# DhayaaAnbajagane/Baryonification

Hardware: AMD Instinct MI355X
Metric: halos/sec for BaryonifyShell NSIDE=1024 (1000000-halo synthetic catalog) (higher is better)
Workload: dtype f64 throughout in the parity-grade mode: f64 ring-row geometry, f64 pair math with 1e-11 elementary functions (fp32 seeds + one Newton step), f64 LDS accumulation, pix_offsets stored as two f32 arrays (hi + lo), f64 regrid geometry, f64 map

## Files before the change

baryonification_amd/csrc/bfgx_api.hip:

```cpp
#include <hip/hip_runtime.h>
#include <cmath>
#include <cstdarg>
#include <cstdio>
#include <algorithm>
#include <climits>
#include <cstdint>
#include <cstdlib>
#include <chrono>
#include <cstring>
#include <functional>
#include <map>
#include <mutex>
#include <string>
#include <tuple>
#include <type_traits>
#include <vector>

#include "../../include/bfgx.h"

#include "bfgx_devmem.hpp"
#include "bfgx_tile_arena.hpp"
#include "bfgx_cosmo.hpp"
#include "bfgx_kernels.hpp"
#include "bfgx_scatter2.hpp"
// ... 65 lines not shown
    for (int d = 0; d < t.ndim; ++d) {
        if (t.n[d] < 2) return fail(BFGX_ERR_INVALID, "table axis %d needs >= 2 points", d);
        if (!t.axis[d]) return fail(BFGX_ERR_INVALID, "table axis %d pointer is NULL", d);
        for (int i = 1; i < t.n[d]; ++i)
            if (!(t.axis[d][i] > t.axis[d][i - 1]))
                return fail(BFGX_ERR_INVALID, "table axis %d must be strictly ascending", d);
    }
    double tot = 1.0;
    for (int d = 0; d < t.ndim; ++d) tot *= t.n[d];
    if (tot > 2.0e9) return fail(BFGX_ERR_INVALID, "table too large for 32-bit row offsets");
    return BFGX_OK;
}

}

struct bfgx_plan {
    int device = 0, num_cus = 256;
    hipStream_t stream = nullptr;
    int64_t nside = 0, max_halos = 0;
    Hpx hpx;
    DevModel model;
    DevList mem;
    HaloRec *recs = nullptr;
    RowSetX *rowsx = nullptr;
    int NC = 4;
    int algo = 1;
    bool blocking_growth = false;
    float *k0_work_est = nullptr;
    int32_t *k1_form = nullptr;
    int64_t k1_nhalos = 0;
    int k1_fluid = 1;
    Tiling tiling;
    TileArena arena;
    int32_t *tile_start = nullptr, *entries = nullptr, *overflow = nullptr;
    int32_t *entries_a = nullptr, *slow_list = nullptr, *slow_cnt = nullptr;
    int32_t entries_a_cap = 0;
    int32_t cnt_pad = 1;
    TileRef *tref = nullptr;
    FarList far;
    int32_t *regrid_lean = nullptr;
    int auto_acc = 0;
    double table_disp_pixels = 0.0;
    int32_t *tile_apron = nullptr;
    int band_reach = 1;
    int route_margin = 0;
    int64_t cat_blk_rows = 0, cat_blk_stride = 0;
    ScanScratch scan;
    bool fast_ok = false;
    RowRec *rowrec = nullptr;
    void *pairrec = nullptr;
    FbRec *fbrec = nullptr;
    const float *tab8f = nullptr;
    const double *tab8d = nullptr;
    unsigned long long *pair_total = nullptr;
    double *tile_sums = nullptr;
    std::vector<int32_t> band_tile0_host;
    int64_t capacity = 0;
    bool timing = false;
    std::vector<std::pair<hipEvent_t, hipEvent_t>> ev[BFGX_NUM_KERNELS];
    std::vector<std::pair<hipEvent_t, hipEvent_t>> ev_free;
};

namespace {

template <class Plan>
struct KernelTimerT {
// ... 122 lines not shown
    float *lo(const void *offsets, int64_t n) const { return split() ? (float *)offsets + 3 * (size_t)n : nullptr; }
    int acc() const { return kind == F32 ? BFGX_ACC_F32 : kind == F64 ? BFGX_ACC_F64 : BFGX_ACC_PARITY; }
};

static int disp_mode(const bfgx_plan *p, int acc, bool one_array, DispMode &m)
{
    if (!p) return fail(BFGX_ERR_INVALID, "NULL plan");
    if (acc != BFGX_ACC_AUTO && acc != BFGX_ACC_F32 && acc != BFGX_ACC_F64 && acc != BFGX_ACC_PARITY)
        return fail(BFGX_ERR_INVALID, "acc_f64 = %d: must be BFGX_ACC_AUTO (-1), 0 (f32), 1 (f64) or BFGX_ACC_PARITY (3)", acc);
    if (acc == BFGX_ACC_AUTO) acc = p->auto_acc;
    const bool parity = acc == BFGX_ACC_PARITY && use_fast(p);
    m.kind = acc == BFGX_ACC_F32 ? DispMode::F32 : (parity && !one_array) ? DispMode::SPLIT : DispMode::F64;
    return BFGX_OK;
}

struct PaintMode {
    enum Kind { F32, F64, MIXED } kind = F64;
    bool map_f64() const { return kind != F32; }
    bool k0_f64() const { return kind == F64; }
    bool pair_f32() const { return kind == MIXED; }
};

static int paint_mode(const bfgx_plan *p, int acc, PaintMode &m)
{
    if (!p) return fail(BFGX_ERR_INVALID, "NULL plan");
    if (acc < 0 || acc > 2) return fail(BFGX_ERR_INVALID, "acc_f64 must be 0, 1 or 2");
    m.kind = acc == 0 ? PaintMode::F32 : (acc == 2 && use_fast(p)) ? PaintMode::MIXED : PaintMode::F64;
    return BFGX_OK;
}

struct TileLaunch {
    float *offsets_lo = nullptr;
    bool paint_pair_f32 = false;
    float *omax = nullptr;
    int tile_lo = 0, tile_n = -1;
    int spread_tiles = -1;
};

static int launch_prep(bfgx_plan *p, const bfgx_catalog *c, int fallback4, bool bin, bool f64, bool rec_all)
{
    if (c->n == 0) return BFGX_OK;
    const unsigned grid = (unsigned)((c->n + 255) / 256);
    KernelTimer kt(p, BFGX_K_PREP);
    PrepOut o;
    std::memset(&o, 0, sizeof(o));
    o.rec = p->recs; o.rowsx = p->rowsx;
    o.fast = (bin && use_fast(p)) ? 1 : 0;
    o.rec_all = (rec_all || !o.fast) ? 1 : 0;
    o.rowrec = p->rowrec; o.pairrec = p->pairrec; o.fbrec = p->fbrec;
    if (bin) {
        o.tref = p->tref; o.cnt_a = p->arena.cnt_a_pad; o.cnt_b = p->arena.cnt_b;
        o.cnt_pad = p->cnt_pad;
        o.work_est = o.fast ? p->k0_work_est : nullptr;
        o.entries_a = p->entries_a; o.cap_a = p->entries_a_cap; o.slow_list = p->slow_list; o.slow_cnt = p->slow_cnt;
    }
    o.ncell_m = p->model.tab.n[1] - 1; o.nrm1 = p->model.tab.n[2] - 1;
    o.blk_rows = p->cat_blk_rows; o.blk_stride = p->cat_blk_stride;
    ExtraCols ex;
    for (int k = 0; k < BFGX_MAX_EXTRA; ++k) ex.p[k] = c->extra[k];
#define BFGX_PREP(NCV, REAL)                                                                                        \
    hipLaunchKernelGGL((halo_prep_kernel<NCV, REAL>), dim3(grid), dim3(256), 0, p->stream, p->model, p->hpx, c->n, c->M, c->z, \
                       c->ra, c->dec, ex, c->ln1pz, c->lnM, fallback4, p->tiling, o)
    if (p->NC == 4) { if (f64) BFGX_PREP(4, double); else BFGX_PREP(4, float); }
    else if (p->NC == 8) BFGX_PREP(8, float);
    else if (p->NC == 16) BFGX_PREP(16, float);
    else if (p->NC == 32) BFGX_PREP(32, float);
    else BFGX_PREP(64, float);
#undef BFGX_PREP
    HIP_TRY(hipGetLastError());
    return BFGX_OK;
}

static int launch_place(bfgx_plan *p, const bfgx_catalog *c)
{
    const unsigned grid = (unsigned)((c->n + 255) / 256);
    hipLaunchKernelGGL(tile_place_kernel, dim3(grid), dim3(256), 0, p->stream, p->hpx, p->tiling, c->n,
                       (const TileRef *)p->tref, (const int32_t *)p->tile_start, p->arena.cur_b, p->entries, p->capacity, p->overflow,
                       (const int32_t *)p->slow_list, (const int32_t *)p->slow_cnt);
    HIP_TRY(hipGetLastError());
    return BFGX_OK;
}

static int launch_prep_and_bin(bfgx_plan *p, const bfgx_catalog *c, int fallback4, bool f64)
{
    p->k1_nhalos = c->n;
    HIP_TRY(hipMemsetAsync(p->arena.base, 0, p->arena.zeroed_bytes, p->stream));
    if (int rc = launch_prep(p, c, fallback4, true, f64, false)) return rc;
    KernelTimer kt(p, BFGX_K_BIN);
    const int nt_i = p->tiling.ntiles, nsb = (nt_i + kScanTilesPerWg - 1) / kScanTilesPerWg;
    const int32_t *cnt = p->arena.cnt_b;
    if (nsb <= 1 || nsb > 1024) {
        hipLaunchKernelGGL(tile_scan_kernel, dim3(1), dim3(1024), 0, p->stream, nt_i, cnt, p->tile_start);
    } else {
        int32_t *tot = p->scan.block_tot, *off = p->scan.block_off;
        hipLaunchKernelGGL(tile_scan_part_kernel<0>, dim3(nsb), dim3(1024), 0, p->stream, nt_i, cnt, p->tile_start, tot, (const int32_t *)off);
        hipLaunchKernelGGL(tile_scan_blocks_kernel, dim3(1), dim3(1024), 0, p->stream, nsb, nt_i, (const int32_t *)tot, off, p->tile_start);
        hipLaunchKernelGGL(tile_scan_part_kernel<1>, dim3(nsb), dim3(1024), 0, p->stream, nt_i, cnt, p->tile_start, tot, (const int32_t *)off);
    }
    HIP_TRY(hipGetLastError());
    if (c->n > 0) if (int rc = launch_place(p, c)) return rc;
    return BFGX_OK;
}

template <int MODE, typename ACC>
static int launch_scatter(bfgx_plan *p, int64_t n, ACC *out, int64_t *counts)
{
    if (n == 0) return BFGX_OK;
    const unsigned grid = (unsigned)((n + kWavesPerBlock - 1) / kWavesPerBlock);
    KernelTimer kt(p, MODE == MODE_OFFSETS ? BFGX_K_OFFSETS : (MODE == MODE_PAINT ? BFGX_K_PAINT : BFGX_K_COUNT));
    hipLaunchKernelGGL((halo_scatter_kernel<MODE, ACC>), dim3(grid), dim3(kWave * kWavesPerBlock), 0, p->stream,
                       make_pair_table(p->model.tab), p->hpx, n, (const HaloRec *)p->recs, out, counts);
    HIP_TRY(hipGetLastError());
    return BFGX_OK;
}

template <int MODE, typename ACC, int NC>
static int launch_tile_scatter_nc(bfgx_plan *p, ACC *out, const TileLaunch &k)
{
    constexpr int NCOMP = (MODE == MODE_OFFSETS) ? 3 : 1;
    const size_t lds = tile_lds_bytes<NC>(p->tiling.BR, p->tiling.W, NCOMP);
    auto kern = tile_scatter_kernel<MODE, ACC, NC>;
    HIP_TRY(hipFuncSetAttribute((const void *)kern, hipFuncAttributeMaxDynamicSharedMemorySize, (int)lds));
    KernelTimer kt(p, MODE == MODE_OFFSETS ? BFGX_K_OFFSETS : (MODE == MODE_PAINT ? BFGX_K_PAINT : BFGX_K_COUNT));
    const int grid = k.tile_n < 0 ? p->tiling.ntiles : std::max(k.tile_n, 1);
    hipLaunchKernelGGL(kern, dim3(grid), dim3(kWave * kWavesPerBlock), lds, p->stream,
                       make_pair_table(p->model.tab), p->hpx, p->tiling, (const HaloRec *)p->recs, (const RowSetX *)p->rowsx,
                       (const int32_t *)p->tile_start, (const int32_t *)p->entries, p->capacity, out, p->pair_total,
                       (unsigned int *)k.omax, k.tile_lo, k.tile_n);
    HIP_TRY(hipGetLastError());
    return BFGX_OK;
}

template <int MODE, typename ACC, typename real, int PM = 0>
static int launch_tile_scatter2(bfgx_plan *p, ACC *out, const TileLaunch &k, ACC *out_lo = nullptr)
{
    constexpr int NCOMP = (MODE == MODE_OFFSETS) ? 3 : 1;
    constexpr int kNP = 1;
    const size_t lds = tile2_lds_bytes<real>(p->tiling.BR, p->tiling.W, NCOMP);
    auto kern = tile_scatter2_kernel<MODE, ACC, real, kNP, PM>;
    HIP_TRY(hipFuncSetAttribute((const void *)kern, hipFuncAttributeMaxDynamicSharedMemorySize, (int)lds));
    Tab8T<real> tb;
    tb.v = (sizeof(real) == 4) ? (const real *)p->tab8f : (const real *)p->tab8d;
    tb.r0 = (real)p->model.tab.r0; tb.r1 = (real)p->model.tab.r1; tb.inv_dr = (real)p->model.tab.inv_dr;
    tb.nr = p->model.tab.n[2]; tb._pad = 0;
    unsigned int *tile_counter = p->arena.tile_counter;
    const int ntodo = k.tile_n < 0 ? p->tiling.ntiles : std::max(k.tile_n, 1);
    KernelTimer kt(p, MODE == MODE_OFFSETS ? BFGX_K_OFFSETS : (MODE == MODE_PAINT ? BFGX_K_PAINT : BFGX_K_COUNT));
    int32_t *form = nullptr;
    if constexpr (MODE != MODE_COUNT) {
        const size_t ldsf = tile2f_lds_bytes<real>(p->tiling.BR, p->tiling.W, NCOMP);
        const bool eligible = p->k1_fluid && ldsf <= (size_t)160 * 1024 && p->tiling.BR <= kWave && ntodo >= 2 * p->num_cus;
        const int nspread = k.spread_tiles > 0 ? k.spread_tiles : ntodo;
        const bool dense = (double)p->k1_nhalos * (double)p->tiling.ntiles >= 6.0e5 * (double)nspread;
        const bool forced = p->k1_fluid == 2 && ldsf <= (size_t)160 * 1024 && p->tiling.BR <= kWave;
        if (eligible && !dense && !forced && p->k0_work_est && p->k1_nhalos > 0) {
            const int nblk = (int)((p->k1_nhalos + 255) / 256);
            hipLaunchKernelGGL(k1_form_kernel, dim3(1), dim3(1024), 0, p->stream, nblk, (const float *)p->k0_work_est, 4800.0f * (float)nspread, p->k1_form);
            form = p->k1_form;
        }
        if (forced || (eligible && (dense || form))) {
            auto kf = tile_scatter2f_kernel<MODE, ACC, real, PM>;
            HIP_TRY(hipFuncSetAttribute((const void *)kf, hipFuncAttributeMaxDynamicSharedMemorySize, (int)ldsf));
            const int gridf = std::min(ntodo, p->num_cus);
            hipLaunchKernelGGL(kf, dim3(std::max(gridf, 1)), dim3(kWave * FluidWaves<real>::n), ldsf, p->stream, tb, p->hpx, p->tiling,
                               (const RowRec *)p->rowrec, (const PairRecT<real> *)p->pairrec, (const FbRec *)p->fbrec,
                               (const int32_t *)p->tile_start, (const int32_t *)p->arena.cnt_a_pad, (const int32_t *)p->arena.cnt_b,
                               (const int32_t *)p->entries, p->capacity, (const int32_t *)p->entries_a, (int)p->entries_a_cap, (int)p->cnt_pad, out, out_lo, tile_counter,
                               (unsigned int *)k.omax, k.tile_lo, k.tile_n, p->overflow, (const int32_t *)form, 1);
            HIP_TRY(hipGetLastError());
            if (!form) return BFGX_OK;
        }
    }
    const int grid = std::min(ntodo, 2 * p->num_cus);
    hipLaunchKernelGGL(kern, dim3(grid), dim3(kWave * kW2), lds, p->stream, tb, p->hpx, p->tiling,
                       (const RowRec *)p->rowrec, (const PairRecT<real> *)p->pairrec, (const FbRec *)p->fbrec,
                       (const int32_t *)p->tile_start, (const int32_t *)p->arena.cnt_a_pad, (const int32_t *)p->arena.cnt_b,
                       (const int32_t *)p->entries, p->capacity, (const int32_t *)p->entries_a, (int)p->entries_a_cap, (int)p->cnt_pad, out, out_lo, p->pair_total, tile_counter,
                       (unsigned int *)k.omax, k.tile_lo, k.tile_n, (const int32_t *)form, 0);
    HIP_TRY(hipGetLastError());
    return BFGX_OK;
}

template <int MODE, typename ACC>
static int launch_tile_scatter(bfgx_plan *p, ACC *out, const TileLaunch &k)
{
    if (use_fast(p)) {
        using real = typename std::conditional<sizeof(ACC) == 8, double, float>::type;
        if constexpr (MODE == MODE_OFFSETS && sizeof(ACC) == 4) {
            if (k.offsets_lo) return launch_tile_scatter2<MODE, ACC, double, 1>(p, out, k, (ACC *)k.offsets_lo);
        }
        if constexpr (MODE == MODE_PAINT && sizeof(ACC) == 8) {
            if (k.paint_pair_f32) return launch_tile_scatter2<MODE, ACC, float>(p, out, k);
        }
        return launch_tile_scatter2<MODE, ACC, real>(p, out, k);
    }
    if (p->NC == 4) return launch_tile_scatter_nc<MODE, ACC, 4>(p, out, k);
    if (MODE == MODE_COUNT) return launch_tile_scatter_nc<MODE, ACC, 4>(p, out, k);
    if (p->NC == 8) return launch_tile_scatter_nc<MODE, ACC, 8>(p, out, k);
    if (p->NC == 16) return launch_tile_scatter_nc<MODE, ACC, 16>(p, out, k);
    if (p->NC == 32) return launch_tile_scatter_nc<MODE, ACC, 32>(p, out, k);
    return launch_tile_scatter_nc<MODE, ACC, 64>(p, out, k);
}

static int ensure_entry_capacity(bfgx_plan *p, const bfgx_catalog *c)
{
    int32_t ov = 0, total = 0;
    HIP_TRY(hipMemcpyAsync(&ov, p->overflow, sizeof(ov), hipMemcpyDeviceToHost, p->stream));
    HIP_TRY(hipMemcpyAsync(&total, p->tile_start + p->tiling.ntiles, sizeof(total), hipMemcpyDeviceToHost, p->stream));
    HIP_TRY(hipStreamSynchronize(p->stream));
    if (!(ov & 1)) return BFGX_OK;
    HIP_TRY(p->mem.regrow(p->entries, (size_t)total + 16));
// ... 105 lines not shown
static int plan_init_binning(bfgx_plan *p, const bfgx_table &t, size_t nh)
{
    int BR, W;
    std::vector<int32_t> tile0, nphi, nrmin, tband;
    build_tiling(p->nside, t.log_values != 0, BR, W, tile0, nphi, nrmin, tband);
    Tiling &T = p->tiling;
    T.BR = BR; T.W = W; T.nbands = (int)nphi.size(); T.ntiles = (int)tband.size();
    if (int rc = owned_upload(p->mem, p->stream, tile0, T.band_tile0)) return rc;
    p->band_tile0_host = tile0;
    if (int rc = owned_upload(p->mem, p->stream, nphi, T.band_nphi)) return rc;
    if (int rc = owned_upload(p->mem, p->stream, nrmin, T.band_nrmin)) return rc;
    if (int rc = owned_upload(p->mem, p->stream, tband, T.tile_band)) return rc;
    std::vector<int32_t> order(tband.size());
    {
        std::vector<double> weight(tband.size());
        for (size_t q = 0; q < tband.size(); ++q) { order[q] = (int32_t)q; weight[q] = (double)nrmin[tband[q]] / (double)nphi[tband[q]]; }
        std::stable_sort(order.begin(), order.end(), [&](int32_t x, int32_t y) { return weight[x] > weight[y]; });
    }
    if (int rc = owned_upload(p->mem, p->stream, order, T.tile_order)) return rc;
    {
        RingRec *rings = nullptr;
        const size_t nrec = (size_t)(4 * p->nside + 1);
        if (p->mem.alloc(rings, nrec)) return alloc_fail("ring table");
        hipLaunchKernelGGL(ring_table_kernel, dim3((unsigned)((nrec + 255) / 256)), dim3(256), 0, p->stream, p->hpx, rings);
        if (hipGetLastError() != hipSuccess) return fail(BFGX_ERR_HIP, "ring table launch failed");
        T.rings = rings;
    }
    if (hipStreamSynchronize(p->stream) != hipSuccess) return fail(BFGX_ERR_HIP, "stream sync failed");
    p->capacity = 8 * p->max_halos + 4096;
    if (const char *e = std::getenv("BFGX_K1_FLUID")) p->k1_fluid = std::max(0, std::min(2, std::atoi(e)));
    if (const char *e = std::getenv("BFGX_ENTRY_CAP")) p->capacity = std::max<int64_t>(16, std::atoll(e));
    p->cnt_pad = kCntPadMax;
    while (p->cnt_pad > 1 && (size_t)T.ntiles * p->cnt_pad * sizeof(int32_t) > ((size_t)4 << 20)) p->cnt_pad >>= 1;
    const TileArenaLayout AL = tile_arena_layout((size_t)T.ntiles, (size_t)p->cnt_pad);
    int32_t *arena = nullptr;
    if (p->mem.alloc(arena, AL.total_words) || p->mem.alloc(p->tile_start, (size_t)T.ntiles + 1) ||
        p->mem.alloc(p->entries, (size_t)p->capacity) || p->mem.alloc(p->overflow, 1) || p->mem.alloc(p->pair_total, 1) || p->mem.alloc(p->tref, nh))
        return alloc_fail("binning workspace");
    p->arena.bind(arena, AL);
    const double mean = 1.3 * (double)std::max<int64_t>(p->max_halos, 1) / (double)T.ntiles;
    int cap_a = 64;
    while (cap_a < 32768 && (double)cap_a < (mean > 512.0 ? 4.0 : 16.0) * mean + 64.0) cap_a <<= 1;
    while (cap_a > 64 && (size_t)T.ntiles * cap_a * sizeof(int32_t) > ((size_t)1 << 30)) cap_a >>= 1;
    if (const char *e = std::getenv("BFGX_TILE_LIST_CAP")) cap_a = std::max(1, std::atoi(e));
    const size_t nblk = (nh + 255) / 256;
    if (p->mem.alloc(p->k0_work_est, nblk) || p->mem.alloc(p->k1_form, 4)) return alloc_fail("work estimate");
    if (p->mem.alloc(p->entries_a, (size_t)T.ntiles * cap_a) || p->mem.alloc(p->slow_list, nblk * 256) || p->mem.alloc(p->slow_cnt, nblk))
        return alloc_fail("tile lists");
    p->entries_a_cap = cap_a;
    return BFGX_OK;
}

static int plan_init_regrid(bfgx_plan *p)
{
    const Tiling &T = p->tiling;
    const int64_t npx = p->hpx.npix;
    const int64_t want = p->table_disp_pixels < 0.25 ? npx / 16 : (p->table_disp_pixels < 2.0 ? npx / 2 : 4 * npx);
    p->far.cap = std::min<int64_t>(std::max<int64_t>((int64_t)1 << 20, want), (int64_t)1 << 28);
    if (const char *e = std::getenv("BFGX_FAR_CAP")) p->far.cap = std::max<int64_t>(1024, std::atoll(e));
    if (p->mem.alloc(p->far.pix, (size_t)p->far.cap) || p->mem.alloc(p->far.val, (size_t)p->far.cap) ||
        p->mem.alloc(p->tile_apron, 2 * (size_t)(T.ntiles + 1)))
        return alloc_fail("far list");
    if (p->mem.alloc(p->regrid_lean, (size_t)(T.ntiles + 4))) return alloc_fail("lean tile list");
    if (hipMemsetAsync(p->regrid_lean, 0, sizeof(int32_t) * 4, p->stream) != hipSuccess) return fail(BFGX_ERR_HIP, "hipMemset failed");
    p->far.count = &p->arena.ctrl->far_count;
    p->far.overflow = p->arena.band_overflow;
    if (hipMemsetAsync(p->arena.ctrl, 0, p->arena.tail_bytes, p->stream) != hipSuccess) return fail(BFGX_ERR_HIP, "hipMemset failed");
    return BFGX_OK;
}

}

// ... 386 lines not shown
    if (p->NC != 4) return fail(BFGX_ERR_UNSUPPORTED, "tables with extra parameter axes need algo 1 (LDS tiles)");
    return launch_prep(p, cat, fallback4, false, false, true);
}

static int launch_offsets(bfgx_plan *p, const DispMode &m, void *slice, int64_t p0, int64_t p1, TileLaunch k1)
{
    if (m.split()) k1.offsets_lo = m.lo(slice, p1 - p0) - 3 * p0;
    if (m.kind != DispMode::F64) return launch_tile_scatter<MODE_OFFSETS, float>(p, (float *)slice - 3 * p0, k1);
    return launch_tile_scatter<MODE_OFFSETS, double>(p, (double *)slice - 3 * p0, k1);
}

static int offsets_impl(bfgx_plan *p, const bfgx_catalog *cat, void *offsets_dev, const DispMode &m, const TileLaunch &k1)
{
    if (int rc = check_scatter(p, cat, offsets_dev, false)) return rc;
    if (int rc = launch_k0(p, cat, 1, m.fp64())) return rc;
    if (p->algo == 1) return launch_offsets(p, m, offsets_dev, 0, p->hpx.npix, k1);
    if (m.fp64()) return launch_scatter<MODE_OFFSETS, double>(p, cat->n, (double *)offsets_dev, nullptr);
    return launch_scatter<MODE_OFFSETS, float>(p, cat->n, (float *)offsets_dev, nullptr);
}

int bfgx_offsets_device(bfgx_plan *p, const bfgx_catalog *cat, void *offsets_dev, int acc_f64)
{
    DispMode m;
    if (int rc = disp_mode(p, acc_f64, false, m)) return rc;
    return offsets_impl(p, cat, offsets_dev, m, TileLaunch{});
}

static int offsets_bands(bfgx_plan *p, const bfgx_catalog *cat, int32_t band0, int32_t band1, void *slice, const DispMode &m)
{
    TileLaunch k1;
    k1.tile_lo = p->band_tile0_host[band0];
    k1.tile_n = p->band_tile0_host[band1] - k1.tile_lo;
    if (int rc = launch_k0(p, cat, 1, m.fp64())) return rc;
    k1.omax = p->arena.omax;
    return launch_offsets(p, m, slice, ring_first_pixel(p->hpx, 1 + (int64_t)p->tiling.BR * band0),
                          ring_first_pixel(p->hpx, 1 + (int64_t)p->tiling.BR * band1), k1);
}

int bfgx_offsets_bands_device(bfgx_plan *p, const bfgx_catalog *cat, int32_t band0, int32_t band1, void *offsets_slice_dev, int acc_f64)
{
    if (int rc = check_scatter(p, cat, offsets_slice_dev, false, true, band0, band1)) return rc;
    if (band0 == band1) return BFGX_OK;
    DispMode m;
    if (int rc = disp_mode(p, acc_f64, true, m)) return rc;
    return offsets_bands(p, cat, band0, band1, offsets_slice_dev, m);
}

static int launch_paint(bfgx_plan *p, const PaintMode &m, void *slice, int64_t p0, TileLaunch k3)
{
    k3.paint_pair_f32 = m.pair_f32();
    if (m.map_f64()) return launch_tile_scatter<MODE_PAINT, double>(p, (double *)slice - p0, k3);
    return launch_tile_scatter<MODE_PAINT, float>(p, (float *)slice - p0, k3);
}

int bfgx_paint_bands_device(bfgx_plan *p, const bfgx_catalog *cat, int32_t band0, int32_t band1, void *map_slice_dev, int acc_f64)
{
    if (int rc = check_scatter(p, cat, map_slice_dev, true, true, band0, band1)) return rc;
    if (band0 == band1) return BFGX_OK;
    PaintMode m;
    if (int rc = paint_mode(p, acc_f64, m)) return rc;
    TileLaunch k3;
    k3.tile_lo = p->band_tile0_host[band0];
    k3.tile_n = p->band_tile0_host[band1] - k3.tile_lo;
    if (int rc = launch_k0(p, cat, 0, m.k0_f64())) return rc;
    return launch_paint(p, m, map_slice_dev, ring_first_pixel(p->hpx, 1 + (int64_t)p->tiling.BR * band0), k3);
}

// ... 261 lines not shown
                               (const float *)offsets_dev, map_out_dev);
    }
    }
    HIP_TRY(hipGetLastError());
    if (sums_dev) {
        if (p->algo != 1) {
            KernelTimer kt(p, BFGX_K_SUM);
            HIP_TRY(hipMemsetAsync(sums_dev, 0, 2 * sizeof(double), p->stream));
            hipLaunchKernelGGL(sum2_kernel, dim3(1024), dim3(256), 0, p->stream, p->hpx.npix, map_in_dev,
                               (const double *)map_out_dev, sums_dev);
            HIP_TRY(hipGetLastError());
        }
    }
    return BFGX_OK;
}

int bfgx_regrid_device(bfgx_plan *p, const double *map_in_dev, const void *offsets_dev, int acc_f64,
                       double *map_out_dev, double *sums_dev)
{
    if (!p || !map_in_dev || !offsets_dev || !map_out_dev) return fail(BFGX_ERR_INVALID, "NULL argument");
    DispMode m;
    if (int rc = disp_mode(p, acc_f64, false, m)) return rc;
    return regrid_impl(p, map_in_dev, offsets_dev, m, map_out_dev, sums_dev, false);
}

int bfgx_baryonify_device(bfgx_plan *p, const bfgx_catalog *cat, const double *map_in_dev, void *offsets_work_dev, int acc_f64,
                          double *map_out_dev, double *sums_dev)
{
    if (!p || !map_in_dev || !offsets_work_dev || !map_out_dev) return fail(BFGX_ERR_INVALID, "NULL argument");
    DispMode m;
    if (int rc = disp_mode(p, acc_f64, false, m)) return rc;
    TileLaunch k1;
    const bool fused = p->algo == 1;
    if (fused) k1.omax = p->arena.omax;
    if (int rc = offsets_impl(p, cat, offsets_work_dev, m, k1)) return rc;
    return regrid_impl(p, map_in_dev, offsets_work_dev, m, map_out_dev, sums_dev, fused);
}

int bfgx_count_pairs_device(bfgx_plan *p, const bfgx_catalog *cat, int fallback4, int64_t *counts_dev, int64_t *total_host)
{
    if (int rc = check_catalog(p, cat)) return rc;
    HIP_TRY(hipSetDevice(p->device));
    if (p->algo == 1 && !counts_dev) {
        HIP_TRY(hipMemsetAsync(p->pair_total, 0, sizeof(unsigned long long), p->stream));
        if (int rc = launch_prep_and_bin(p, cat, fallback4, false)) return rc;
        if (int rc = launch_tile_scatter<MODE_COUNT, float>(p, (float *)nullptr, TileLaunch{})) return rc;
        unsigned long long tot = 0;
        HIP_TRY(hipMemcpyAsync(&tot, p->pair_total, sizeof(tot), hipMemcpyDeviceToHost, p->stream));
        HIP_TRY(hipStreamSynchronize(p->stream));
        if (total_host) *total_host = (int64_t)tot;
        return bfgx_plan_status(p);
    }
    int64_t *counts = counts_dev;
    DevBuf tmp;
    if (!counts) {
        HIP_TRY(tmp.alloc(sizeof(int64_t) * (size_t)(cat->n > 0 ? cat->n : 1)));
        counts = tmp.as<int64_t>();
    }
    int rc = launch_prep(p, cat, fallback4, false, false, true);
    if (!rc) rc = launch_scatter<MODE_COUNT, float>(p, cat->n, (float *)nullptr, counts);
    if (!rc && total_host) {
        std::vector<int64_t> h((size_t)cat->n);
        if (hipMemcpyAsync(h.data(), counts, sizeof(int64_t) * (size_t)cat->n, hipMemcpyDeviceToHost, p->stream) != hipSuccess ||
            hipStreamSynchronize(p->stream) != hipSuccess)
            rc = fail(BFGX_ERR_HIP, "count copy-back failed");
        else {
            int64_t tot = 0;
// ... 293 lines not shown
    *out = nullptr;
    if (bfgx_device_count() <= 0) return fail(BFGX_ERR_NO_DEVICE, "no HIP device visible");
    HIP_TRY(hipHostMalloc(out, bytes ? bytes : 1, hipHostMallocDefault));
    return BFGX_OK;
}

void bfgx_host_free(void *p) { if (p) (void)hipHostFree(p); }

int bfgx_baryonify_shell(const bfgx_catalog *cat, const bfgx_model *model, int64_t nside,
                         const double *map_in, double *map_out, const bfgx_opts *opts, bfgx_stats *stats)
{
    if (!cat || !model || !map_in || !map_out) return fail(BFGX_ERR_INVALID, "NULL argument");
    const bfgx_opts o = entry_opts(opts);
    std::lock_guard<std::mutex> lk(g_shells.mu);
    ShellEntry *e = nullptr;
    if (int rc = shell_begin(cat, model, nside, o, &e)) return rc;
    bfgx_plan *p = e->plan;
    OneShotCall call(&p->stream, e);
    const size_t npix = (size_t)p->hpx.npix;
    DispMode m;
    if (int rc = disp_mode(p, o.acc_offsets_f64, false, m)) return rc;
    const size_t acc_bytes = npix * m.pixel_bytes();
    std::vector<double> hostlog;
    bfgx_catalog dcat;
    if (int rc = call.mark(0, p->stream)) return rc;
    if (int rc = upload_catalog_pooled(e, cat, &dcat, hostlog, o.catalog_token)) return rc;
    if (e->in.need(npix * sizeof(double)) || e->out.need(npix * sizeof(double)) || e->off.need(acc_bytes) || e->sums.need(40 * sizeof(double)))
        return alloc_fail("map buffers");
    if (o.algo == 0) {
        HIP_TRY(hipMemsetAsync(e->off.p, 0, acc_bytes, p->stream));
        HIP_TRY(hipMemsetAsync(e->out.p, 0, npix * sizeof(double), p->stream));
    }
    TileLaunch k1;
    if (o.algo == 1) k1.omax = p->arena.omax;
    if (int rc = offsets_impl(p, &dcat, e->off.p, m, k1)) return rc;
    double sums[2] = {0, 0};
    Chunks ch;
    chunk_plan(p, o.algo == 1, pipe_knobs(), ch);
    int64_t first_unsent = 0;
    int rc = kOnePass;
    if (ch.piped && call.open(map_in, npix * sizeof(double), map_out, npix * sizeof(double), ch.stage)) {
        map_in = call.src<double>(); map_out = call.dst<double>();
        rc = shell_streamed(call, e, m, ch, sums, &first_unsent);
    }
    if (rc == kOnePass) rc = shell_one_pass(call, e, m, o.algo == 1, map_in, map_out, first_unsent, sums);
    if (rc) return rc;
    if (int rc = bfgx_plan_status(p)) return rc;
    call.commit();
    if (int rc = call.finish(stats, sums, -1)) return rc;
    return o.check_mass ? check_mass(sums[0], sums[1]) : BFGX_OK;
}

int bfgx_paint_shell(const bfgx_catalog *cat, const bfgx_model *model, int64_t nside,
                     double *map_out, const bfgx_opts *opts, bfgx_stats *stats)
{
    if (!cat || !model || !map_out) return fail(BFGX_ERR_INVALID, "NULL argument");
    const bfgx_opts o = entry_opts(opts);
    std::lock_guard<std::mutex> lk(g_shells.mu);
    ShellEntry *e = nullptr;
    if (int rc = shell_begin(cat, model, nside, o, &e)) return rc;
    bfgx_plan *p = e->plan;
    OneShotCall call(&p->stream, e);
    PaintMode m;
    if (int rc = paint_mode(p, o.acc_paint_f64, m)) return rc;

    const size_t npix = (size_t)p->hpx.npix;
    std::vector<double> hostlog;
// ... 176 lines not shown
```

baryonification_amd/csrc/bfgx_kernels.hpp:

```cpp
#pragma once
#include <hip/hip_runtime.h>
#include <stdint.h>
#include "bfgx_cosmo.hpp"
#include "bfgx_math.hpp"

namespace bfgx {

constexpr double kTwoPi    = 6.283185307179586476925286766559005768394;
constexpr double kHalfPi   = 1.570796326794896619231321691639751442099;
constexpr double kInvTwoPi = 1.0 / kTwoPi;
constexpr double kTwoThird = 2.0 / 3.0;
constexpr double kDeg2Rad  = kPi / 180.0;
constexpr double kRad2Deg  = 180.0 / kPi;

constexpr int kWave = 64;
constexpr int kWavesPerBlock = 4;
constexpr int kNC = 4;

enum { MODE_OFFSETS = 0, MODE_PAINT = 1, MODE_COUNT = 2 };

struct Hpx {
    int64_t nside, npix, ncap;
    double fact1, fact2;
};
// ... 455 lines not shown
__device__ inline RunSlot wave_run_issue(int32_t *cnt, int tile, bool active)
{
    RunSlot r;
    r.base = 0; r.hr = 0;
    if (__ballot(active) == 0ull) return r;
    const int lane = (int)__builtin_amdgcn_mbcnt_hi(~0u, __builtin_amdgcn_mbcnt_lo(~0u, 0u));
    const int key = active ? tile : -1 - lane;
    const int prev = __shfl_up(key, 1, kWave);
    const bool head = (lane == 0) || (key != prev);
    const unsigned long long hm = __ballot(head);
    const int hl = 63 - __clzll((long long)(hm & ((2ull << lane) - 1ull)));
    const unsigned long long up = (lane == kWave - 1) ? 0ull : (hm >> (lane + 1));
    const int next = up ? lane + __ffsll((long long)up) : kWave;
    r.hr = active ? (hl | ((lane - hl + 1) << 8)) : 0;
    if (head && active) r.base = atomicAdd(cnt + tile, next - lane);
    return r;
}
__device__ inline int wave_run_resolve(const RunSlot &r)
{
    const int b = __shfl(r.base, r.hr & 63, kWave);
    return r.hr ? b + (r.hr >> 8) - 1 : 0;
}

struct PrepOut {
    HaloRec *rec;
    RowSetX *rowsx;
    RowRec *rowrec;
    void *pairrec;
    FbRec *fbrec;
    TileRef *tref;
    int32_t *cnt_a, *cnt_b;
    int32_t *entries_a, *slow_list, *slow_cnt;
    float *work_est;
    int32_t cap_a;
    int32_t cnt_pad;
    int32_t fast;
    int32_t rec_all;
    int32_t ncell_m, nrm1;
    int64_t blk_rows, blk_stride;
};

template <int NC, typename real>
__device__ __forceinline__ void halo_prep_one(const DevModel &m, const Hpx &h, int64_t j, bool live, const double *gz, const double *gm,
                                              const double *__restrict__ M, const double *__restrict__ z,
                                              const double *__restrict__ ra, const double *__restrict__ dec,
                                              ExtraCols ex,
                                              const double *__restrict__ lnz1, const double *__restrict__ lnM,
                                              int fallback4, const Tiling &T, const PrepOut &o, int *s_nslow, float *s_work);

constexpr int kK0Occ = 4;
template <int NC, typename real>
__global__ void __launch_bounds__(256, kK0Occ)
halo_prep_kernel(DevModel m, Hpx h, int64_t nhalo,
                 const double *__restrict__ M, const double *__restrict__ z,
                 const double *__restrict__ ra, const double *__restrict__ dec,
                 ExtraCols ex,
                 const double *__restrict__ lnz1, const double *__restrict__ lnM,
                 int fallback4, Tiling T, PrepOut o)
{
    __shared__ int s_nslow;
    __shared__ float s_work;
    if (threadIdx.x == 0) { s_nslow = 0; s_work = 0.0f; }
    constexpr int kAxisLds = 128;
    __shared__ double ax_lds[2 * kAxisLds];
    const bool ax_in_lds = m.tab.n[0] <= kAxisLds && m.tab.n[1] <= kAxisLds;
    if (ax_in_lds) {
        for (int i = threadIdx.x; i < m.tab.n[0]; i += blockDim.x) ax_lds[i] = m.tab.axis[0][i];
        for (int i = threadIdx.x; i < m.tab.n[1]; i += blockDim.x) ax_lds[kAxisLds + i] = m.tab.axis[1][i];
        __syncthreads();
    }
    const double *gz = ax_in_lds ? ax_lds : m.tab.axis[0], *gm = ax_in_lds ? ax_lds + kAxisLds : m.tab.axis[1];
    constexpr int kBandLds = 1024;
    __shared__ int32_t band_lds[3 * kBandLds + 1];
    if (o.tref && T.nbands <= kBandLds) {
        for (int i = threadIdx.x; i <= T.nbands; i += blockDim.x) band_lds[i] = T.band_tile0[i];
        for (int i = threadIdx.x; i < T.nbands; i += blockDim.x) { band_lds[kBandLds + 1 + i] = T.band_nphi[i]; band_lds[2 * kBandLds + 1 + i] = T.band_nrmin[i]; }
        __syncthreads();
        T.band_tile0 = band_lds; T.band_nphi = band_lds + kBandLds + 1; T.band_nrmin = band_lds + 2 * kBandLds + 1;
    }
    __syncthreads();
    const int64_t j = (int64_t)blockIdx.x * blockDim.x + threadIdx.x;
    halo_prep_one<NC, real>(m, h, j < nhalo ? j : nhalo - 1, j < nhalo, gz, gm, M, z, ra, dec, ex, lnz1, lnM, fallback4, T, o, &s_nslow, &s_work);
    if (o.slow_cnt) {
        __syncthreads();
        if (threadIdx.x == 0) o.slow_cnt[blockIdx.x] = s_nslow;
        if (threadIdx.x == 0 && o.work_est) o.work_est[blockIdx.x] = s_work;
    }
}

template <int NC, typename real>
__device__ __forceinline__ void halo_prep_one(const DevModel &m, const Hpx &h, int64_t j, bool live, const double *gz, const double *gm,
                                              const double *__restrict__ M, const double *__restrict__ z,
                                              const double *__restrict__ ra, const double *__restrict__ dec,
                                              ExtraCols ex,
                                              const double *__restrict__ lnz1, const double *__restrict__ lnM,
// ... 1283 lines not shown
```

baryonification_amd/csrc/bfgx_tile_arena.hpp:

```cpp
#pragma once
#include <cstddef>
#include <cstdint>

namespace bfgx {

struct RegridCtrl {
    unsigned long long far_count;
    int32_t far_overflow_full;
    int32_t todo_count;
};
static_assert(sizeof(RegridCtrl) == 16 && alignof(RegridCtrl) == 8, "RegridCtrl is four words, the first two a 64-bit counter");

constexpr size_t kCtrlWords = sizeof(RegridCtrl) / sizeof(int32_t);
constexpr size_t round_up4(size_t words) { return (words + 3) & ~(size_t)3; }

struct TileArenaLayout {
    size_t cnt_a_pad, cnt_b, cur_b, tile_counter, omax, ctrl, far_overflow_full, todo, todo_list, band_overflow;
    size_t cursor_words;
    size_t zeroed_words;
    size_t tail_words;
    size_t total_words;
};

constexpr TileArenaLayout tile_arena_layout(size_t ntiles, size_t cnt_pad)
{
    const size_t blk = ntiles + 1;
    TileArenaLayout L{};
    L.cnt_a_pad = 0;
    L.cnt_b = round_up4(ntiles * cnt_pad);
    L.cur_b = L.cnt_b + blk;
    L.tile_counter = L.cur_b + blk;
    L.omax = L.tile_counter + 1;
    L.ctrl = L.cnt_b + round_up4(L.omax + blk - L.cnt_b);
    L.far_overflow_full = L.ctrl + offsetof(RegridCtrl, far_overflow_full) / sizeof(int32_t);
    L.todo = L.ctrl + offsetof(RegridCtrl, todo_count) / sizeof(int32_t);
    L.todo_list = L.ctrl + kCtrlWords;
    L.band_overflow = L.todo_list + ntiles;
    L.cursor_words = L.tile_counter - L.cur_b;
    L.zeroed_words = L.ctrl + kCtrlWords;
    L.total_words = L.band_overflow + 4;
    L.tail_words = L.total_words - L.ctrl;
    return L;
}

struct TileArena {
    int32_t *base = nullptr;
    int32_t *cnt_a_pad = nullptr, *cnt_b = nullptr, *cur_b = nullptr;
    unsigned int *tile_counter = nullptr;
    float *omax = nullptr;
    RegridCtrl *ctrl = nullptr;
    int32_t *far_overflow_full = nullptr;
    int32_t *todo = nullptr;
    int32_t *band_overflow = nullptr;
    size_t cursor_bytes = 0, zeroed_bytes = 0, tail_bytes = 0;

    void bind(int32_t *b, const TileArenaLayout &L)
    {
        base = b;
        cnt_a_pad = b + L.cnt_a_pad; cnt_b = b + L.cnt_b; cur_b = b + L.cur_b;
        tile_counter = (unsigned int *)(b + L.tile_counter);
        omax = (float *)(b + L.omax);
        ctrl = (RegridCtrl *)(b + L.ctrl);
        far_overflow_full = b + L.far_overflow_full;
        todo = b + L.todo;
        band_overflow = b + L.band_overflow;
        cursor_bytes = sizeof(int32_t) * L.cursor_words;
        zeroed_bytes = sizeof(int32_t) * L.zeroed_words;
        tail_bytes = sizeof(int32_t) * L.tail_words;
    }
};

constexpr size_t kScanBlocksRoom = 1024;
struct ScanScratchLayout { size_t block_tot, block_off, total_words; };
constexpr ScanScratchLayout scan_scratch_layout()
{
    ScanScratchLayout L{};
    L.block_tot = 0;
    L.block_off = L.block_tot + kScanBlocksRoom;
    L.total_words = L.block_off + kScanBlocksRoom;
    return L;
}
struct ScanScratch {
    int32_t *block_tot = nullptr, *block_off = nullptr;
    void bind(int32_t *b, const ScanScratchLayout &L) { block_tot = b + L.block_tot; block_off = b + L.block_off; }
};

template <size_t NT, size_t PAD>
struct TileArenaCheck {
    static constexpr TileArenaLayout L = tile_arena_layout(NT, PAD);
    static constexpr size_t blk = NT + 1;
    static constexpr bool unrounded = (NT * PAD) % 4 == 0;
    static constexpr size_t n3p = round_up4(3 * blk + 1);
    static_assert(L.cnt_a_pad == 0 && L.cnt_b >= NT * PAD, "the padded counters start the arena and hold ntiles * cnt_pad words");
    static_assert(L.cur_b == L.cnt_b + blk && L.cursor_words == blk && L.tile_counter == L.cur_b + L.cursor_words,
                  "cnt_b and cur_b: ntiles + 1 words each, and nothing else lies in the cursors' span");
    static_assert(L.omax == L.tile_counter + 1, "the |offset|^2 block follows the tile counter");
    static_assert(L.ctrl >= L.omax + blk && L.ctrl - (L.omax + blk) < 4, "the control words follow the three blocks and the tile counter, rounded up to four words");
    static_assert(L.far_overflow_full == L.ctrl + 2 && L.todo == L.ctrl + 3 && L.todo_list == L.todo + 1, "count (64 bits), overflow, todo count, todo tiles");
    static_assert(L.band_overflow == L.todo_list + NT && L.total_words > L.band_overflow, "the banded overflow flag follows the todo tiles, inside the allocation");
    static_assert(L.zeroed_words == L.ctrl + kCtrlWords, "the zeroed span starts at the base and ends exactly after RegridCtrl");
    static_assert(L.zeroed_words % 4 == 0, "the zeroed span is a multiple of 16 bytes");
    static_assert(L.todo_list >= L.zeroed_words && L.band_overflow >= L.zeroed_words, "the step's memset touches neither the todo tiles nor the banded overflow flag");
    static_assert(L.ctrl % 2 == 0, "RegridCtrl's 64-bit counter is 8-byte aligned (the base is a device allocation)");
    static_assert(L.tail_words == L.total_words - L.ctrl && L.tail_words == NT + 8, "plan creation zeroes the control words and all behind them");
    static_assert(L.cnt_b == round_up4(NT * PAD) && (!unrounded || L.cnt_b == NT * PAD), "only a padded region that is no multiple of four words is rounded up");
    static_assert(L.tile_counter == L.cnt_b + 2 * blk && L.omax == L.cnt_b + 2 * blk + 1 && L.ctrl == L.cnt_b + n3p, "the three blocks, the tile counter between the second and the third");
    static_assert(L.zeroed_words == L.cnt_b + n3p + 4 && L.total_words == L.cnt_b + n3p + NT + 8, "lengths of the memset and of the allocation");
    static constexpr bool ok = true;
};
static_assert(TileArenaCheck<1, 32>::ok && TileArenaCheck<2, 32>::ok && TileArenaCheck<14, 32>::ok && TileArenaCheck<52, 32>::ok &&
              TileArenaCheck<6208, 32>::ok && TileArenaCheck<98560, 8>::ok && TileArenaCheck<393728, 2>::ok &&
              TileArenaCheck<3, 1>::ok && TileArenaCheck<12289, 1>::ok, "tile arena layout");

static_assert(scan_scratch_layout().block_tot == 0 && scan_scratch_layout().block_off == 1024 && scan_scratch_layout().total_words == 2048,
              "scan scratch: 1024 totals, then 1024 offsets: one word each per scan block");

}
```

Baseline: 923.2 million.

## Double-buffer tile arena and zero the spare copy inside the prep kernel

Allocates two tile arenas and, on each step, has the halo prep kernel zero the idle arena with a grid-stride loop. The next step then swaps to the pre-zeroed arena instead of issuing a hipMemsetAsync. This removes one memset launch per step from the critical path. The cost is twice the arena memory, extra stores inside prep, and added state (the band_overflow flag is pinned to the first arena) that has to stay consistent across steps.

```diff
diff --git a/baryonification_amd/csrc/bfgx_api.hip b/baryonification_amd/csrc/bfgx_api.hip
--- a/baryonification_amd/csrc/bfgx_api.hip
+++ b/baryonification_amd/csrc/bfgx_api.hip
@@ -121,6 +121,11 @@
     int k1_fluid = 1;
     Tiling tiling;
     TileArena arena;
+    TileArenaLayout arena_layout{};
+    int32_t *arena_mem[2] = {nullptr, nullptr};
+    int arena_bound = 0;
+    bool spare_zero = false;
+    bool step_fold = true;
     int32_t *tile_start = nullptr, *entries = nullptr, *overflow = nullptr;
     int32_t *entries_a = nullptr, *slow_list = nullptr, *slow_cnt = nullptr;
     int32_t entries_a_cap = 0;
@@ -309,12 +314,12 @@
 struct TileLaunch {
     float *offsets_lo = nullptr;
     bool paint_pair_f32 = false;
-    float *omax = nullptr;
+    bool omax = false;
     int tile_lo = 0, tile_n = -1;
     int spread_tiles = -1;
 };
 
-static int launch_prep(bfgx_plan *p, const bfgx_catalog *c, int fallback4, bool bin, bool f64, bool rec_all)
+static int launch_prep(bfgx_plan *p, const bfgx_catalog *c, int fallback4, bool bin, bool f64, bool rec_all, bool zero_spare = false)
 {
     if (c->n == 0) return BFGX_OK;
     const unsigned grid = (unsigned)((c->n + 255) / 256);
@@ -330,6 +335,10 @@
         o.cnt_pad = p->cnt_pad;
         o.work_est = o.fast ? p->k0_work_est : nullptr;
         o.entries_a = p->entries_a; o.cap_a = p->entries_a_cap; o.slow_list = p->slow_list; o.slow_cnt = p->slow_cnt;
+        if (zero_spare) {
+            o.zero = (int4 *)p->arena_mem[1 - p->arena_bound];
+            o.zero_n = (int32_t)(p->arena.zeroed_bytes / 16);
+        }
     }
     o.ncell_m = p->model.tab.n[1] - 1; o.nrm1 = p->model.tab.n[2] - 1;
     o.blk_rows = p->cat_blk_rows; o.blk_stride = p->cat_blk_stride;
@@ -358,11 +367,25 @@
     return BFGX_OK;
 }
 
+static void bind_arena(bfgx_plan *p, int which)
+{
+    p->arena_bound = which;
+    p->arena.bind(p->arena_mem[which], p->arena_layout, p->arena_mem[0]);
+    p->far.count = &p->arena.ctrl->far_count;
+}
+
+constexpr int64_t kZeroPiecesPerThread = 4;
+
 static int launch_prep_and_bin(bfgx_plan *p, const bfgx_catalog *c, int fallback4, bool f64)
 {
     p->k1_nhalos = c->n;
-    HIP_TRY(hipMemsetAsync(p->arena.base, 0, p->arena.zeroed_bytes, p->stream));
-    if (int rc = launch_prep(p, c, fallback4, true, f64, false)) return rc;
+    const int64_t k0_threads = ((c->n + 255) / 256) * 256;
+    const bool k0_zeroes = p->step_fold && (int64_t)(p->arena.zeroed_bytes / 16) <= kZeroPiecesPerThread * k0_threads;
+    const bool spare_was_zero = p->spare_zero;
+    p->spare_zero = false;
+    if (spare_was_zero) bind_arena(p, 1 - p->arena_bound);
+    else HIP_TRY(hipMemsetAsync(p->arena.base, 0, p->arena.zeroed_bytes, p->stream));
+    if (int rc = launch_prep(p, c, fallback4, true, f64, false, k0_zeroes)) return rc;
     KernelTimer kt(p, BFGX_K_BIN);
     const int nt_i = p->tiling.ntiles, nsb = (nt_i + kScanTilesPerWg - 1) / kScanTilesPerWg;
     const int32_t *cnt = p->arena.cnt_b;
@@ -376,6 +399,7 @@
     }
     HIP_TRY(hipGetLastError());
     if (c->n > 0) if (int rc = launch_place(p, c)) return rc;
+    p->spare_zero = k0_zeroes;
     return BFGX_OK;
 }
 
@@ -403,7 +427,7 @@
     hipLaunchKernelGGL(kern, dim3(grid), dim3(kWave * kWavesPerBlock), lds, p->stream,
                        make_pair_table(p->model.tab), p->hpx, p->tiling, (const HaloRec *)p->recs, (const RowSetX *)p->rowsx,
                        (const int32_t *)p->tile_start, (const int32_t *)p->entries, p->capacity, out, p->pair_total,
-                       (unsigned int *)k.omax, k.tile_lo, k.tile_n);
+                       k.omax ? (unsigned int *)p->arena.omax : nullptr, k.tile_lo, k.tile_n);
     HIP_TRY(hipGetLastError());
     return BFGX_OK;
 }
@@ -443,7 +467,7 @@
                                (const RowRec *)p->rowrec, (const PairRecT<real> *)p->pairrec, (const FbRec *)p->fbrec,
                                (const int32_t *)p->tile_start, (const int32_t *)p->arena.cnt_a_pad, (const int32_t *)p->arena.cnt_b,
                                (const int32_t *)p->entries, p->capacity, (const int32_t *)p->entries_a, (int)p->entries_a_cap, (int)p->cnt_pad, out, out_lo, tile_counter,
-                               (unsigned int *)k.omax, k.tile_lo, k.tile_n, p->overflow, (const int32_t *)form, 1);
+                               k.omax ? (unsigned int *)p->arena.omax : nullptr, k.tile_lo, k.tile_n, p->overflow, (const int32_t *)form, 1);
             HIP_TRY(hipGetLastError());
             if (!form) return BFGX_OK;
         }
@@ -453,7 +477,7 @@
                        (const RowRec *)p->rowrec, (const PairRecT<real> *)p->pairrec, (const FbRec *)p->fbrec,
                        (const int32_t *)p->tile_start, (const int32_t *)p->arena.cnt_a_pad, (const int32_t *)p->arena.cnt_b,
                        (const int32_t *)p->entries, p->capacity, (const int32_t *)p->entries_a, (int)p->entries_a_cap, (int)p->cnt_pad, out, out_lo, p->pair_total, tile_counter,
-                       (unsigned int *)k.omax, k.tile_lo, k.tile_n, (const int32_t *)form, 0);
+                       k.omax ? (unsigned int *)p->arena.omax : nullptr, k.tile_lo, k.tile_n, (const int32_t *)form, 0);
     HIP_TRY(hipGetLastError());
     return BFGX_OK;
 }
@@ -625,12 +649,17 @@
     if (const char *e = std::getenv("BFGX_ENTRY_CAP")) p->capacity = std::max<int64_t>(16, std::atoll(e));
     p->cnt_pad = kCntPadMax;
     while (p->cnt_pad > 1 && (size_t)T.ntiles * p->cnt_pad * sizeof(int32_t) > ((size_t)4 << 20)) p->cnt_pad >>= 1;
+    if (const char *e = std::getenv("BFGX_STEP_FOLD")) p->step_fold = std::atoi(e) != 0;
     const TileArenaLayout AL = tile_arena_layout((size_t)T.ntiles, (size_t)p->cnt_pad);
+    const size_t arena_stride = tile_arena_stride(AL);
     int32_t *arena = nullptr;
-    if (p->mem.alloc(arena, AL.total_words) || p->mem.alloc(p->tile_start, (size_t)T.ntiles + 1) ||
+    if (p->mem.alloc(arena, 2 * arena_stride) || p->mem.alloc(p->tile_start, (size_t)T.ntiles + 1) ||
         p->mem.alloc(p->entries, (size_t)p->capacity) || p->mem.alloc(p->overflow, 1) || p->mem.alloc(p->pair_total, 1) || p->mem.alloc(p->tref, nh))
         return alloc_fail("binning workspace");
-    p->arena.bind(arena, AL);
+    if (hipMemsetAsync(arena, 0, sizeof(int32_t) * 2 * arena_stride, p->stream) != hipSuccess) return fail(BFGX_ERR_HIP, "hipMemset failed");
+    p->arena_layout = AL;
+    p->arena_mem[0] = arena; p->arena_mem[1] = arena + arena_stride;
+    bind_arena(p, 0);
     const double mean = 1.3 * (double)std::max<int64_t>(p->max_halos, 1) / (double)T.ntiles;
     int cap_a = 64;
     while (cap_a < 32768 && (double)cap_a < (mean > 512.0 ? 4.0 : 16.0) * mean + 64.0) cap_a <<= 1;
@@ -1083,7 +1112,7 @@
     k1.tile_lo = p->band_tile0_host[band0];
     k1.tile_n = p->band_tile0_host[band1] - k1.tile_lo;
     if (int rc = launch_k0(p, cat, 1, m.fp64())) return rc;
-    k1.omax = p->arena.omax;
+    k1.omax = true;
     return launch_offsets(p, m, slice, ring_first_pixel(p->hpx, 1 + (int64_t)p->tiling.BR * band0),
                           ring_first_pixel(p->hpx, 1 + (int64_t)p->tiling.BR * band1), k1);
 }
@@ -1411,7 +1440,7 @@
     if (int rc = disp_mode(p, acc_f64, false, m)) return rc;
     TileLaunch k1;
     const bool fused = p->algo == 1;
-    if (fused) k1.omax = p->arena.omax;
+    k1.omax = fused;
     if (int rc = offsets_impl(p, cat, offsets_work_dev, m, k1)) return rc;
     return regrid_impl(p, map_in_dev, offsets_work_dev, m, map_out_dev, sums_dev, fused);
 }
@@ -1771,7 +1800,7 @@
         HIP_TRY(hipMemsetAsync(e->out.p, 0, npix * sizeof(double), p->stream));
     }
     TileLaunch k1;
-    if (o.algo == 1) k1.omax = p->arena.omax;
+    k1.omax = o.algo == 1;
     if (int rc = offsets_impl(p, &dcat, e->off.p, m, k1)) return rc;
     double sums[2] = {0, 0};
     Chunks ch;
diff --git a/baryonification_amd/csrc/bfgx_kernels.hpp b/baryonification_amd/csrc/bfgx_kernels.hpp
--- a/baryonification_amd/csrc/bfgx_kernels.hpp
+++ b/baryonification_amd/csrc/bfgx_kernels.hpp
@@ -511,6 +511,8 @@
     int32_t *cnt_a, *cnt_b;
     int32_t *entries_a, *slow_list, *slow_cnt;
     float *work_est;
+    int4 *zero;
+    int32_t zero_n;
     int32_t cap_a;
     int32_t cnt_pad;
     int32_t fast;
@@ -540,6 +542,9 @@
     __shared__ int s_nslow;
     __shared__ float s_work;
     if (threadIdx.x == 0) { s_nslow = 0; s_work = 0.0f; }
+    if (o.zero)
+        for (int64_t i = (int64_t)blockIdx.x * blockDim.x + threadIdx.x; i < o.zero_n; i += (int64_t)gridDim.x * blockDim.x)
+            o.zero[i] = make_int4(0, 0, 0, 0);
     constexpr int kAxisLds = 128;
     __shared__ double ax_lds[2 * kAxisLds];
     const bool ax_in_lds = m.tab.n[0] <= kAxisLds && m.tab.n[1] <= kAxisLds;
diff --git a/baryonification_amd/csrc/bfgx_tile_arena.hpp b/baryonification_amd/csrc/bfgx_tile_arena.hpp
--- a/baryonification_amd/csrc/bfgx_tile_arena.hpp
+++ b/baryonification_amd/csrc/bfgx_tile_arena.hpp
@@ -42,6 +42,7 @@
     L.tail_words = L.total_words - L.ctrl;
     return L;
 }
+constexpr size_t tile_arena_stride(const TileArenaLayout &L) { return round_up4(L.total_words); }
 
 struct TileArena {
     int32_t *base = nullptr;
@@ -54,7 +55,7 @@
     int32_t *band_overflow = nullptr;
     size_t cursor_bytes = 0, zeroed_bytes = 0, tail_bytes = 0;
 
-    void bind(int32_t *b, const TileArenaLayout &L)
+    void bind(int32_t *b, const TileArenaLayout &L, int32_t *first)
     {
         base = b;
         cnt_a_pad = b + L.cnt_a_pad; cnt_b = b + L.cnt_b; cur_b = b + L.cur_b;
@@ -63,7 +64,7 @@
         ctrl = (RegridCtrl *)(b + L.ctrl);
         far_overflow_full = b + L.far_overflow_full;
         todo = b + L.todo;
-        band_overflow = b + L.band_overflow;
+        band_overflow = first + L.band_overflow;
         cursor_bytes = sizeof(int32_t) * L.cursor_words;
         zeroed_bytes = sizeof(int32_t) * L.zeroed_words;
         tail_bytes = sizeof(int32_t) * L.tail_words;
@@ -100,6 +101,7 @@
     static_assert(L.band_overflow == L.todo_list + NT && L.total_words > L.band_overflow, "the banded overflow flag follows the todo tiles, inside the allocation");
     static_assert(L.zeroed_words == L.ctrl + kCtrlWords, "the zeroed span starts at the base and ends exactly after RegridCtrl");
     static_assert(L.zeroed_words % 4 == 0, "the zeroed span is a multiple of 16 bytes");
+    static_assert(tile_arena_stride(L) % 4 == 0 && tile_arena_stride(L) >= L.total_words, "the second arena starts 16-byte aligned behind the first");
     static_assert(L.todo_list >= L.zeroed_words && L.band_overflow >= L.zeroed_words, "the step's memset touches neither the todo tiles nor the banded overflow flag");
     static_assert(L.ctrl % 2 == 0, "RegridCtrl's 64-bit counter is 8-byte aligned (the base is a device allocation)");
     static_assert(L.tail_words == L.total_words - L.ctrl && L.tail_words == NT + 8, "plan creation zeroes the control words and all behind them");
```

Result: no change. 924.4 million, median of 2 (+0.1%).
